# mindspore-lab/minddiffusion

Hardware: AMD Instinct MI355X
Metric: 512x512 txt2img latents/sec (50-step DDIM) (higher is better)
Workload: dtype f16; 1 GPU; SDv2 txt2img 512x512 (64x64 latent), 50-step DDIM, CFG 9.0, batch 1 per GPU (BASELINE.json configs[1]); synthetic seeded weights + synthetic text conditioning; global_batch=1, parallelism=batch-shard x1, hip_graph=True, rccl_world_size=1, broadcast_bytes=0, ddim_steps=50, unet_batch_per_gpu=2, sampler=ddim, cfg_dup_prefix=False

## Files before the change

include/mdx.h:

```cpp
#ifndef MDX_H_
#define MDX_H_

#include <stddef.h>
#include <stdint.h>

#ifdef __cplusplus
extern "C" {
#endif

#define MDX_OK 0
#define MDX_E_INVALID (-1)
#define MDX_E_WORKSPACE (-2)
#define MDX_E_HIP (-3)

typedef void* mdx_stream_t;

int mdx_version(void);
const char* mdx_last_error(void);
int mdx_set_option(const char* name, int value);
int mdx_get_option(const char* name, int* value);

int mdx_nchw_to_nhwc_f16(const float* x, void* y, int B, int C, int H, int W, int Cpad, mdx_stream_t s);
int mdx_nhwc_to_nchw_f32(const void* x, float* y, int B, int C, int H, int W, int Cstride, mdx_stream_t s);

// ... 101 lines not shown

int mdx_groupnorm_from_splitk_f16(const mdx_gemm_desc* prod, const float* gamma, const float* beta, void* y, int groups,
                                  float eps, int silu, mdx_stream_t s);
int mdx_groupnorm_from_splitk_ok(const mdx_gemm_desc* prod, int groups);

int mdx_attention_f16(const void* q, long q_bs, int q_ld, const void* k, long k_bs, int k_ld, const void* vt,
                      long vt_bs, int vt_ld, void* o, long o_bs, int o_ld, int B, int heads, int D, int Nq, int Nk,
                      float scale, mdx_stream_t s);

size_t mdx_attention_ws_bytes(int B, int heads, int D, int Nq, int Nk);
int mdx_attention_splitkv_f16(const void* q, long q_bs, int q_ld, const void* k, long k_bs, int k_ld, const void* vt,
                              long vt_bs, int vt_ld, void* o, long o_bs, int o_ld, int B, int heads, int D, int Nq, int Nk,
                              float scale, int kv_splits, void* ws, size_t ws_bytes, mdx_stream_t s);

typedef struct mdx_st_tail_desc {
    const void* attn_out;
    const void* tok;
    const void* x_in;
    void* out;
    const void* ctx_k;
    const void* ctx_vt;
    const void* wstream;
    const float* vec;
    float* colstats_out;
    void* debug_out;
    int debug_stage;
    int B, tokens;
    int C, heads, dim_head;
    int ctx_len, ctx_cap;
    float scale;
    float ln_eps;
    int tile_rows;
    int warm;
} mdx_st_tail_desc;
#define MDX_ST_DEBUG_COUNT_BARRIERS 100
int mdx_st_tail_sched_barriers(int C, int tile_rows);
int mdx_st_head_sched_barriers(int C, int tile_rows);
int mdx_st_tail_f16(const mdx_st_tail_desc* d, mdx_stream_t s);
int mdx_st_tail_supported(int C, int heads, int dim_head, int tokens_per_sample, int tile_rows);
size_t mdx_st_tail_stream_bytes(int C);

typedef struct mdx_st_head_desc {
    const void* x;
    const float* colstats;
    int nrb;
    const void* wstream;
    const float* vec;
    void* tok;
    void* qk;
    void* vt;
    int vt_ld;
    void* debug_out;
    int debug_stage;
    int B, tokens, C;
    float gn_eps, ln_eps;
    int tile_rows;
    int warm;
} mdx_st_head_desc;
int mdx_st_head_f16(const mdx_st_head_desc* d, mdx_stream_t s);
int mdx_st_head_supported(int C, int tokens_per_sample, int tile_rows);
size_t mdx_st_head_stream_bytes(int C);

int mdx_timestep_embedding_f32(const float* t, float* out, int M, int dim, float max_period, mdx_stream_t s);

int mdx_dense_small_f32(const float* x, int x_ld, const void* w, const float* b, float* out, int out_ld, int M,
                        int N, int K, int act_in, int act_out, mdx_stream_t s);
// ... 143 lines not shown
```

minddiffusion_amd/_lib.py:

```python
import ctypes
import os

_HERE = os.path.dirname(os.path.abspath(__file__))
LIB_PATH = os.environ.get("MDX_LIBRARY") or os.path.join(_HERE, "libmdx.so")

c_void_p = ctypes.c_void_p
c_int = ctypes.c_int
c_uint = ctypes.c_uint
c_long = ctypes.c_long
c_float = ctypes.c_float
c_size_t = ctypes.c_size_t


class MdxError(RuntimeError):
    pass


class GemmDesc(ctypes.Structure):
    _fields_ = [
        ("a", c_void_p), ("a2", c_void_p), ("c1", c_int), ("c2", c_int),
        ("w", c_void_p), ("bias", c_void_p), ("rowbias", c_void_p), ("rowbias_ld", c_int),
        ("residual", c_void_p), ("residual_ld", c_int),
        ("out", c_void_p), ("out_ld", c_int),
        ("B", c_int), ("H", c_int), ("W", c_int), ("N", c_int),
        ("ksize", c_int), ("stride", c_int), ("upsample", c_int),
        ("epilogue", c_int), ("out_mode", c_int), ("splitk", c_int),
        ("workspace", c_void_p), ("workspace_bytes", c_size_t),
        ("out_bs", c_long),
        ("out2", c_void_p), ("out2_ld", c_int), ("n_split", c_int), ("asym_pad", c_int),
        ("stats_out", c_void_p), ("ln_stats", c_void_p), ("ln_s", c_void_p), ("ln_nt", c_int), ("ln_eps", c_float),
        ("colstats_out", c_void_p), ("colstats_cap", c_int), ("defer_reduce", c_int),
        ("tile_m", c_int), ("tile_n", c_int),
        ("gn_colstats", c_void_p), ("gn_gamma", c_void_p), ("gn_beta", c_void_p), ("gn_nrb", c_int), ("gn_silu", c_int),
        ("gn_eps", c_float),
        ("skip_a", c_void_p), ("skip_a2", c_void_p), ("skip_c1", c_int), ("skip_c2", c_int), ("skip_w", c_void_p),
        ("w_frag", c_int), ("stages", c_int), ("w_sub", c_void_p),
        ("xattn_k", c_void_p), ("xattn_vt", c_void_p), ("xattn_len", c_int), ("xattn_cap", c_int), ("xattn_scale", c_float),
        ("act_slope", c_void_p), ("act_slope_n", c_int),
        ("geglu_unit", c_int),
    ]


class StTailDesc(ctypes.Structure):
    _fields_ = [
        ("attn_out", c_void_p), ("tok", c_void_p), ("x_in", c_void_p), ("out", c_void_p),
        ("ctx_k", c_void_p), ("ctx_vt", c_void_p), ("wstream", c_void_p), ("vec", c_void_p),
        ("colstats_out", c_void_p), ("debug_out", c_void_p), ("debug_stage", c_int),
        ("B", c_int), ("tokens", c_int), ("C", c_int), ("heads", c_int), ("dim_head", c_int),
        ("ctx_len", c_int), ("ctx_cap", c_int), ("scale", c_float), ("ln_eps", c_float), ("tile_rows", c_int), ("warm", c_int),
    ]


class StHeadDesc(ctypes.Structure):
    _fields_ = [
        ("x", c_void_p), ("colstats", c_void_p), ("nrb", c_int), ("wstream", c_void_p), ("vec", c_void_p),
        ("tok", c_void_p), ("qk", c_void_p), ("vt", c_void_p), ("vt_ld", c_int), ("debug_out", c_void_p), ("debug_stage", c_int),
        ("B", c_int), ("tokens", c_int), ("C", c_int), ("gn_eps", c_float), ("ln_eps", c_float), ("tile_rows", c_int),
        ("warm", c_int),
    ]


class LoraMergeDesc(ctypes.Structure):
    _fields_ = [
        ("base", c_void_p), ("A", c_void_p), ("B", c_void_p), ("N", c_int), ("K", c_int), ("R", c_int), ("scale", c_float),
        ("gamma", c_void_p), ("beta", c_void_p), ("bias", c_void_p), ("S", c_void_p), ("cb", c_void_p),
        ("dst", c_void_p), ("layout", c_int), ("ld", c_int), ("dst_n0", c_int), ("dst_N", c_int),
        ("piece_stride", c_int), ("piece_offset", c_int),
    ]


EPI_NONE, EPI_GEGLU, EPI_GELU, EPI_QUICKGELU, EPI_PRELU = 0, 1, 2, 3, 4
OUT_ROWMAJOR, OUT_TRANSPOSED, OUT_D2S2 = 0, 1, 2
LORA_ROWMAJOR, LORA_TILED, LORA_FRAG = 0, 1, 2

SIGNATURES = {
    "mdx_version": (c_int, []),
    "mdx_last_error": (ctypes.c_char_p, []),
    "mdx_set_option": (c_int, [ctypes.c_char_p, c_int]),
    "mdx_get_option": (c_int, [ctypes.c_char_p, ctypes.POINTER(c_int)]),
    "mdx_nchw_to_nhwc_f16": (c_int, [c_void_p, c_void_p, c_int, c_int, c_int, c_int, c_int, c_void_p]),
    "mdx_nhwc_to_nchw_f32": (c_int, [c_void_p, c_void_p, c_int, c_int, c_int, c_int, c_int, c_void_p]),
    "mdx_groupnorm_ws_floats": (c_size_t, [c_int, c_int, c_int, c_int]),
# ... 143 lines not shown
```

minddiffusion_amd/csrc/attention.hip:

```cpp
#include "mdx_common.h"

#include <type_traits>
#include <utility>

namespace {

struct AttnParams {
    const f16* q;
    const f16* k;
    const f16* vt;
    f16* o;
    long q_bs, k_bs, vt_bs, o_bs;
    int q_ld, k_ld, vt_ld, o_ld;
    int B, heads, Nq, Nk;
    float scale_log2;
    unsigned k_bytes, vt_bytes;
    int causal;
    int nsplit, qblocks;
    char* ws_part;
    unsigned* tickets;
    int fast_stage;
};

constexpr int BQ = 128;
// ... 852 lines not shown
template <int D, int OCC>
void launch_attn(const AttnParams& p, dim3 grid, hipStream_t st) {
    constexpr int KS = (D + 15) / 16, DT = (D + 31) / 32;
    constexpr int KCH = (2 * KS <= 8) ? 8 : (2 * KS <= 16 ? 16 : 32);
    constexpr size_t stage = (size_t)BKV * KCH * 16 + (size_t)DT * 32 * 128;
    constexpr size_t ostage = (size_t)4 * 32 * (DT * 32 + 8) * 2 + 16;
    constexpr size_t lds = (2 * stage > ostage ? 2 * stage : ostage);
    static MdxPerDeviceOnce attr_once;
    if (attr_once.first()) {
        (void)hipFuncSetAttribute(reinterpret_cast<const void*>(&attn_kernel<D, OCC>),
                                  hipFuncAttributeMaxDynamicSharedMemorySize, (int)lds);
    }
    hipLaunchKernelGGL((attn_kernel<D, OCC>), grid, dim3(256), lds, st, p);
}

constexpr int ATTN_MAX_SPLITS = ATTN_MAX_SPLITS_K;

int attn_cus() {
    static int cus[64] = {};
    int dv = 0;
    if (hipGetDevice(&dv) != hipSuccess || dv < 0 || dv >= 64) return 256;
    if (!cus[dv]) {
        int n = 0;
        cus[dv] = (hipDeviceGetAttribute(&n, hipDeviceAttributeMultiprocessorCount, dv) == hipSuccess && n > 0) ? n : 256;
    }
    return cus[dv];
}

int attn_blocks_per_cu(int D) { return D <= 64 ? (mdx_opt(MDX_OPT_ATTN_OCC3) ? 3 : 2) : (D <= 80 ? 2 : 1); }

int attn_auto_splits(int B, int heads, int D, int Nq, int Nk) {
    const int mode = mdx_opt(MDX_OPT_ATTN_KV_SPLIT);
    const int ntiles = (Nk + BKV - 1) / BKV;
    int cap = mode >= 2 ? ntiles / 2 : ntiles / 24;
    if (cap > ATTN_MAX_SPLITS) cap = ATTN_MAX_SPLITS;
    if (mode == 0 || cap < 2) return 1;
    if (mode >= 2) return mode < cap ? mode : cap;
    const long items = (long)((Nq + BQ - 1) / BQ) * heads * B;
    const long slots = (long)attn_cus() * attn_blocks_per_cu(D);
    long s = slots / items;
    if (s > cap) s = cap;
    return s < 2 ? 1 : (int)s;
}

constexpr long ATTN_TICKET_ITEMS = 16384;
constexpr size_t ATTN_TICKET_BYTES = (size_t)ATTN_TICKET_ITEMS * 4;
size_t attn_part_bytes(int D) { return (size_t)BQ * D * 2 + (size_t)BQ * 8; }

}

static int attention_impl(const void* q, long q_bs, int q_ld, const void* k, long k_bs, int k_ld, const void* vt,
                          long vt_bs, int vt_ld, void* o, long o_bs, int o_ld, int B, int heads, int D, int Nq, int Nk,
                          float scale, int causal, int kv_splits, void* ws, size_t ws_bytes, mdx_stream_t s) {
    MDX_REQUIRE(q && k && vt && o, "mdx_attention_f16: null pointer");
    MDX_REQUIRE(D == 40 || D == 64 || D == 80 || D == 160, "mdx_attention_f16: head dim %d not supported (40/64/80/160)", D);
    MDX_REQUIRE(B > 0 && heads > 0 && Nq > 0 && Nk > 0, "mdx_attention_f16: bad extents");
    MDX_REQUIRE(q_ld % 8 == 0 && k_ld % 8 == 0 && vt_ld % 8 == 0 && o_ld % 8 == 0, "mdx_attention_f16: strides must be multiples of 8");
    MDX_REQUIRE(vt_ld >= Nk, "mdx_attention_f16: vt_ld < Nk");
    AttnParams p{};
    p.q = (const f16*)q;
    p.k = (const f16*)k;
    p.vt = (const f16*)vt;
    p.o = (f16*)o;
    p.q_bs = q_bs; p.k_bs = k_bs; p.vt_bs = vt_bs; p.o_bs = o_bs;
    p.q_ld = q_ld; p.k_ld = k_ld; p.vt_ld = vt_ld; p.o_ld = o_ld;
    p.B = B; p.heads = heads; p.Nq = Nq; p.Nk = Nk;
    p.scale_log2 = scale * 1.4426950408889634f;
    p.causal = causal;
    const size_t kbytes = ((size_t)(Nk - 1) * k_ld + D) * 2;
    const size_t vbytes = ((size_t)(D - 1) * vt_ld + vt_ld) * 2;
    MDX_REQUIRE(kbytes <= 0x80000000ull && vbytes <= 0x80000000ull, "mdx_attention_f16: K/V extent too large");
// ... 97 lines not shown
```

minddiffusion_amd/csrc/stchain.hip:

```cpp
#include "mdx_common.h"

namespace {

typedef unsigned u32x4 __attribute__((ext_vector_type(4)));

struct StTailParams {
    const f16* attn_o;
    const f16* tok;
    const f16* x_in;
    f16* out;
    const f16* kc;
    const f16* vtc;
    const char* wstream;
    const float* vec;
    float* colstats_out;
    f16* dbg;
    int M, HW, TC, ctx_len, heads, nshare, lead;
    float scale_log2, eps;
    int stop_after;
    unsigned wstream_bytes, kc_bytes, vtc_bytes;
};

constexpr int PF = 10;

__device__ __forceinline__ void lds_barrier() {
    asm volatile("s_waitcnt lgkmcnt(0)\n\ts_barrier" ::: "memory");
}

#define LDS_BARRIER() do { lds_barrier(); ++nbar; } while (0)
constexpr int ST_COUNT_BARRIERS = 100;

__device__ __forceinline__ u32x4 wload(const __amdgpu_buffer_rsrc_t rs, unsigned voff, unsigned piece) {
    return __builtin_amdgcn_raw_buffer_load_b128(rs, voff, piece * 1024u, 0);
}

template <int C, int TM, int T>
__device__ __forceinline__ void unit(f32x16 (&acc)[T][TM], const char* abuf_lane, u32x4 (&ring)[PF],
                                     const __amdgpu_buffer_rsrc_t rs, const unsigned voff, unsigned& piece) {
    constexpr int KS = C / 16;
    constexpr int LDB = (C + 8) * 2;
    static_assert((KS * T) % PF == 0, "ring position must be 0 at every unit boundary");
    constexpr int AD = 2;
    f16x8 af[AD + 1][TM];
    f32x16 odd;
#pragma unroll
    for (int r = 0; r < 16; ++r) odd[r] = 0.f;
#pragma unroll
    for (int s = 0; s < AD; ++s)
#pragma unroll
        for (int i = 0; i < TM; ++i) af[s][i] = *reinterpret_cast<const f16x8*>(abuf_lane + i * 32 * LDB + s * 32);
    __builtin_amdgcn_sched_barrier(0);
#pragma unroll
    for (int s = 0; s < KS; ++s) {
// ... 194 lines not shown
                if (dd < D)
                    *reinterpret_cast<f16x4*>(Ab + (rt * 32 + l31) * LDB + (h * D + dd) * 2) =
                        f16x4{(f16)(acc_o[j][4 * g] * inv), (f16)(acc_o[j][4 * g + 1] * inv), (f16)(acc_o[j][4 * g + 2] * inv),
                              (f16)(acc_o[j][4 * g + 3] * inv)};
            }
    }
}

template <int C, int TM, int D, bool LONG>
__global__ __launch_bounds__((C / 32 + 1) * 64) void st_tail_kernel(const StTailParams p) {
    mdx_kernarg_touch<sizeof(StTailParams)>();
    constexpr int NW = C / 32;
    constexpr int NT = NW * 64;
    constexpr int BM = 32 * TM;
    constexpr int LDW = C + 8;
    constexpr int LDB = LDW * 2;
    constexpr int BUF = BM * LDB;
    constexpr int CPR = C / 8;
    constexpr int NH = (TM == 1) ? 2 : 1;
    using V = VecOff<C>;
    extern __shared__ __attribute__((aligned(16))) char smem[];
    char* Xb = smem;
    char* Ab = smem + BUF;
    char* Hb = smem + 2 * BUF;
    float* vec = reinterpret_cast<float*>(smem + (2 + NH) * BUF);
    float2* part = reinterpret_cast<float2*>(vec + V::total);

    int nbar = 0;
    const int tid = threadIdx.x;
    const int lane = tid & 63;
    const int wave = __builtin_amdgcn_readfirstlane(tid >> 6);
    const int hi = lane >> 5, l31 = lane & 31;
    const int m0 = blockIdx.x * BM;
    const int n0 = wave * 32;

    const __amdgpu_buffer_rsrc_t rs_w = make_rsrc(p.wstream, p.wstream_bytes);
    constexpr unsigned PIECES = 3 * (C / 16) + 4 * 3 * (C / 16) + (C / 16);
    if (wave == NW) {
        if (p.nshare <= 0) return;
        constexpr BarSched S = make_sched<C / 16, NH>();
        warmer_wave<NW, PIECES>(p.wstream, S, p.nshare, (unsigned)p.lead, lane);
        return;
    }
    unsigned piece = (unsigned)wave * PIECES;
    const unsigned voff = (unsigned)lane * 16u;
    u32x4 ring[PF];
#pragma unroll
    for (int j = 0; j < PF; ++j) ring[j] = wload(rs_w, voff, piece + j);

    {
        const f16* ga = p.attn_o + (size_t)m0 * C;
        const f16* gx = p.tok + (size_t)m0 * C;
        for (int idx = tid; idx < BM * CPR; idx += NT) {
            const int row = idx / CPR, ch = idx - row * CPR;
            const f16x8 va = *reinterpret_cast<const f16x8*>(ga + (size_t)row * C + ch * 8);
            const f16x8 vx = *reinterpret_cast<const f16x8*>(gx + (size_t)row * C + ch * 8);
            *reinterpret_cast<f16x8*>(Ab + row * LDB + ch * 16) = va;
            *reinterpret_cast<f16x8*>(Xb + row * LDB + ch * 16) = vx;
        }
        for (int idx = tid; idx < V::total / 4; idx += NT)
            reinterpret_cast<float4*>(vec)[idx] = reinterpret_cast<const float4*>(p.vec)[idx];
    }
    LDS_BARRIER();

    const int lane_row_off = l31 * LDB + hi * 16;
    const int epi_off = l31 * LDB + (n0 + 4 * hi) * 2;

    auto dump = [&](const char* buf) {
        LDS_BARRIER();
        for (int idx = tid; idx < BM * CPR; idx += NT) {
            const int row = idx / CPR, ch = idx - row * CPR;
            *reinterpret_cast<f16x8*>(p.dbg + (size_t)(m0 + row) * C + ch * 8) =
                *reinterpret_cast<const f16x8*>(buf + row * LDB + ch * 16);
        }
    };

    auto residual_ln = [&](f32x16 (&acc)[1][TM], const float* bias, const float* gamma, const float* beta) {
        f16x4 th[TM][4];
#pragma unroll
        for (int i = 0; i < TM; ++i) {
            float su = 0.f, sq = 0.f;
#pragma unroll
            for (int g = 0; g < 4; ++g) {
                const float4 bb = *reinterpret_cast<const float4*>(bias + n0 + 8 * g + 4 * hi);
                const f16x4 xr = *reinterpret_cast<const f16x4*>(Xb + epi_off + i * 32 * LDB + g * 16);
// ... 156 lines not shown
    zero_acc(acc1);
    unit<C, TM, 1>(acc1, Ab + lane_row_off, ring, rs_w, voff, piece);
    residual_ln(acc1, vec + V::bo2, vec + V::g3, vec + V::be3);
    if (p.stop_after == 5) { dump(Xb); return; }
    if (p.stop_after == 6) { dump(Ab); return; }

    f32x16 acc2[1][TM];
    zero_acc(acc2);
#pragma unroll 1
    for (int c = 0; c < 4; ++c) {
        f32x16 accg[2][TM];
        zero_acc(accg);
        unit<C, TM, 2>(accg, Ab + lane_row_off, ring, rs_w, voff, piece);
        const float* ba = vec + V::b1 + c * C + n0 + 4 * hi;
        const float* bg = ba + 4 * C;
#pragma unroll
        for (int i = 0; i < TM; ++i)
#pragma unroll
            for (int g = 0; g < 4; ++g) {
                const float4 a4 = *reinterpret_cast<const float4*>(ba + 8 * g);
                const float4 g4 = *reinterpret_cast<const float4*>(bg + 8 * g);
                const float aa[4] = {a4.x, a4.y, a4.z, a4.w}, gg[4] = {g4.x, g4.y, g4.z, g4.w};
                f16x4 hv;
#pragma unroll
                for (int e = 0; e < 4; ++e) hv[e] = (f16)((accg[0][i][4 * g + e] + aa[e]) * gelu_tanh_f(accg[1][i][4 * g + e] + gg[e]));
                *reinterpret_cast<f16x4*>(Hb + (c % NH) * BUF + epi_off + i * 32 * LDB + g * 16) = hv;
            }
        LDS_BARRIER();
        unit<C, TM, 1>(acc2, Hb + (c % NH) * BUF + lane_row_off, ring, rs_w, voff, piece);
        if (NH == 1) LDS_BARRIER();
    }
    {
        f16x8 xin[(BM * CPR + NT - 1) / NT];
        const f16* gx = p.x_in + (size_t)m0 * C;
#pragma unroll
        for (int k = 0; k < (BM * CPR + NT - 1) / NT; ++k) {
            const int idx = tid + k * NT;
            if (idx < BM * CPR) {
                const int row = idx / CPR, ch = idx - row * CPR;
                xin[k] = *reinterpret_cast<const f16x8*>(gx + (size_t)row * C + ch * 8);
            }
        }
#pragma unroll
        for (int i = 0; i < TM; ++i)
#pragma unroll
            for (int g = 0; g < 4; ++g) {
                const float4 bb = *reinterpret_cast<const float4*>(vec + V::b2 + n0 + 8 * g + 4 * hi);
                const f16x4 xr = *reinterpret_cast<const f16x4*>(Xb + epi_off + i * 32 * LDB + g * 16);
                const float b4[4] = {bb.x, bb.y, bb.z, bb.w};
                f16x4 tv;
#pragma unroll
                for (int e = 0; e < 4; ++e) tv[e] = (f16)(acc2[0][i][4 * g + e] + b4[e] + (float)xr[e]);
                *reinterpret_cast<f16x4*>(Ab + epi_off + i * 32 * LDB + g * 16) = tv;
            }
        LDS_BARRIER();
#pragma unroll
        for (int k = 0; k < (BM * CPR + NT - 1) / NT; ++k) {
            const int idx = tid + k * NT;
            if (idx < BM * CPR) {
                const int row = idx / CPR, ch = idx - row * CPR;
                *reinterpret_cast<f16x8*>(Xb + row * LDB + ch * 16) = xin[k];
            }
        }
    }
    if (p.stop_after == 7) { dump(Ab); return; }

    zero_acc(acc1);
// ... 304 lines not shown
    }
    if (p.stop_after == ST_COUNT_BARRIERS && blockIdx.x == 0 && tid == 0) *reinterpret_cast<int*>(p.dbg) = nbar;
}

template <int C, int TM>
void launch_head(const StHeadParams& p, hipStream_t st) {
    constexpr int NW = C / 32, BM = 32 * TM;
    constexpr size_t lds = (size_t)3 * BM * (C + 8) * 2 + (size_t)5 * C * 4 + (size_t)C * 8 + (size_t)NW * BM * 8;
    static_assert(lds <= 160 * 1024, "LDS budget");
    static MdxPerDeviceOnce attr_once;
    if (attr_once.first()) {
        (void)hipFuncSetAttribute(reinterpret_cast<const void*>(&st_head_kernel<C, TM>),
                                  hipFuncAttributeMaxDynamicSharedMemorySize, (int)lds);
    }
    hipLaunchKernelGGL((st_head_kernel<C, TM>), dim3(p.M / BM), dim3((NW + 1) * 64), lds, st, p);
}
}

extern "C" size_t mdx_st_tail_stream_bytes(int C) { return (size_t)(C / 32) * (16 * (C / 16)) * 1024; }

extern "C" int mdx_st_tail_supported(int C, int heads, int dim_head, int tokens_per_sample, int tile_rows) {
    return C == 320 && heads * dim_head == C && (dim_head == 64 || dim_head == 40) && (tile_rows == 32 || tile_rows == 64) &&
           tokens_per_sample > 0 && tokens_per_sample % tile_rows == 0;
}

extern "C" int mdx_st_tail_f16(const mdx_st_tail_desc* d, mdx_stream_t s) {
    MDX_REQUIRE(d && d->attn_out && d->tok && d->x_in && d->out && d->ctx_k && d->ctx_vt && d->wstream && d->vec,
                "mdx_st_tail_f16: null pointer");
    MDX_REQUIRE(mdx_st_tail_supported(d->C, d->heads, d->dim_head, d->tokens, d->tile_rows),
                "mdx_st_tail_f16: unsupported shape C=%d heads=%d d=%d tokens=%d tile_rows=%d", d->C, d->heads, d->dim_head,
                d->tokens, d->tile_rows);
    MDX_REQUIRE(d->B > 0 && d->ctx_len > 0 && d->ctx_len <= d->ctx_cap && d->ctx_cap % 8 == 0 && d->ctx_cap <= 1024,
                "mdx_st_tail_f16: context length %d / capacity %d (capacity: multiple of 8, <= 1024)", d->ctx_len, d->ctx_cap);
    MDX_REQUIRE(d->out != d->attn_out && d->out != d->tok && d->out != d->x_in, "mdx_st_tail_f16: out must not alias an input");
    StTailParams p{};
    p.attn_o = (const f16*)d->attn_out;
    p.tok = (const f16*)d->tok;
    p.x_in = (const f16*)d->x_in;
    p.out = (f16*)d->out;
    p.kc = (const f16*)d->ctx_k;
    p.vtc = (const f16*)d->ctx_vt;
    p.wstream = (const char*)d->wstream;
    p.vec = d->vec;
    p.colstats_out = d->colstats_out;
    p.dbg = (f16*)d->debug_out;
    p.M = d->B * d->tokens;
    p.HW = d->tokens;
    p.TC = d->ctx_cap;
    p.ctx_len = d->ctx_len;
    p.heads = d->heads;
    {
        const int per_xcd = (p.M / d->tile_rows) / 8;
        p.nshare = (d->debug_out || d->warm == 0 || per_xcd < 4) ? 0 : (per_xcd > 32 ? 32 : per_xcd);
        p.lead = 80;
        if (d->warm > 1) {
            p.lead = d->warm / 100;
            if (p.nshare > 0 && d->warm % 100 > 0 && d->warm % 100 < p.nshare) p.nshare = d->warm % 100;
        }
    }
    p.scale_log2 = d->scale * 1.4426950408889634f;
    p.eps = d->ln_eps;
    p.stop_after = d->debug_out ? d->debug_stage : 0;
    p.wstream_bytes = (unsigned)mdx_st_tail_stream_bytes(d->C);
    p.kc_bytes = (unsigned)((size_t)d->ctx_cap * d->C * 2);
    p.vtc_bytes = (unsigned)((size_t)d->C * d->ctx_cap * 2);
    hipStream_t st = (hipStream_t)s;
    const bool lng = d->ctx_len > 96;
    if (d->dim_head == 64) {
        if (d->tile_rows == 64) { if (lng) launch_tail<320, 2, 64, true>(p, st); else launch_tail<320, 2, 64, false>(p, st); }
        else { if (lng) launch_tail<320, 1, 64, true>(p, st); else launch_tail<320, 1, 64, false>(p, st); }
    } else {
        if (d->tile_rows == 64) { if (lng) launch_tail<320, 2, 40, true>(p, st); else launch_tail<320, 2, 40, false>(p, st); }
        else { if (lng) launch_tail<320, 1, 40, true>(p, st); else launch_tail<320, 1, 40, false>(p, st); }
    }
    MDX_LAUNCH_CHECK("mdx_st_tail_f16");
    return MDX_OK;
}

extern "C" int mdx_st_tail_sched_barriers(int C, int tile_rows) {
// ... 48 lines not shown
```

minddiffusion_amd/ldm/modules/diffusionmodules/openaimodel.py:

```python
import ctypes
import math
import os
import re
import weakref

import torch

from .... import ops
from ...._lib import MdxError
from ....planner import PlanBuilder, round_up, capture_or_eager
from ....loader import WeightLoader, named_layers

f16, f32 = torch.float16, torch.float32

LORA_PREFIXES = ("tk_delta_", "mindpet_delta_")
_LORA_KEY = re.compile(r"^(.*)\.(" + "|".join(LORA_PREFIXES) + r")lora_([ab])$")
_LORA_TARGETS = ("to_q", "to_k", "to_v", "to_out.0")


def is_lora_key(name):
    return _LORA_KEY.match(name) is not None


class UNetModel:
# ... 491 lines not shown
        B, C, H, W = x.shape
        if C != self.in_channels:
            raise MdxError(f"UNetModel: expected {self.in_channels} input channels, got {C}")
        if context is None:
            if getattr(self, "_selfctx_bad", None) is None:
                self._selfctx_bad = sorted({l[2] * l[3] for _, l in named_layers(self)
                                            if l[0] == "st" and l[2] * l[3] != self.context_dim})
            bad = self._selfctx_bad
            if bad:
                raise MdxError(f"UNetModel: context=None makes attn2 attend to its own input (attention.py:133), which needs "
                               f"context_dim == transformer width; context_dim={self.context_dim}, widths {bad}")
            P = self._plan(B, H, W, _selfctx=True)
        else:
            P = self._plan(B, H, W)
            self._ensure_context(P, context)
        P.x_static.copy_(x)
        if temb is not None:
            if temb.shape[-1] != self._emb_total or temb.dtype != f32:
                raise MdxError(f"UNetModel: temb must be fp32 [.., {self._emb_total}] rows of time_embedding_table()")
            P.emb_all.copy_(temb)
        else:
            P.t_static.copy_(timesteps.to(device=self.device, dtype=f32) if isinstance(timesteps, torch.Tensor)
                             else torch.as_tensor(timesteps, dtype=f32, device=self.device))
            if y is not None:
                yy = torch.as_tensor(y).to(device=self.device, dtype=torch.long).reshape(-1)
                if yy.shape[0] != B:
                    raise MdxError(f"UNetModel: y has {yy.shape[0]} labels for a batch of {B}")
                if int(yy.min()) < 0 or int(yy.max()) >= self.num_classes:
                    raise MdxError(f"UNetModel: class label outside [0, {self.num_classes})")
                P.y_static.copy_(yy)
            for op in P.main[:P.temb_ops]:
                op()
        dup = self._dup_body(P) if (cfg_dup and context is not None and y is None) else None
        if dup is not None and ops.get_option("unet_cfg_dup_check"):
            hb = B // 2
            same = torch.equal(P.x_static[:hb], P.x_static[hb:]) and torch.equal(P.emb_all[:hb], P.emb_all[hb:])
            if not same:
                raise MdxError("UNetModel: cfg_dup=True, but the two halves of the batch do not carry the same x / timesteps")
        if self.use_graph and not P.graph_failed:
            if dup is not None:
                if P.dup_graph is None:
                    self._capture(P, dup)
                if P.dup_graph is not None:
                    P.dup_graph.replay()
                    return P.eps_nhwc
            if P.graph is None:
                self._capture(P)
            if P.graph is not None:
                P.graph.replay()
                return P.eps_nhwc
        body = dup if dup is not None else P.main[P.temb_ops:]
        for op in body:
            op()
        self.last_launch_count = P.temb_ops + len(body)
        return P.eps_nhwc

    def _dup_body(self, P):
        mn = ops.get_option("unet_cfg_dup")
        if not mn or P.B < mn or P.B % 2 or P.ck is None:
            return None
        if hasattr(P, "dup_body"):
            return P.dup_body
        P.dup_body = None
        h = P.B // 2
        PA = self._plan(h, P.H, P.W)
        if PA.ck is None:
            return None
        late = "op2" in P.ck and "op2" in PA.ck and len(P.ck["live2"]) == len(PA.ck["live2"])
        ko, kl = ("op2", "live2") if late else ("op", "live")
        ib, ic = P.main.index(P.ck[ko]), P.main.index(P.ck["conv_in"])
        ja, jc = PA.main.index(PA.ck[ko]), PA.main.index(PA.ck["conv_in"])
        xin_a, xin_b = PA.ck["xin"], P.ck["xin"]
        copies = [lambda: xin_a.copy_(xin_b[:h]), lambda: PA.emb_all.copy_(P.emb_all[:h])]
        spread = []
        for src, dst in zip(PA.ck[kl], P.ck[kl]):
            if not (dst.shape[0] == 2 * src.shape[0] and dst.shape[1:] == src.shape[1:] and dst.dtype == src.dtype):
                raise MdxError(f"UNetModel: guidance-duplicate prefix: live tensors of the two plans do not pair up "
                               f"({tuple(src.shape)} vs {tuple(dst.shape)})")
            spread.append(lambda src=src, dst=dst, k=src.shape[0]: (dst[:k].copy_(src), dst[k:].copy_(src)))
        P.dup_half = PA
        P.dup_body = P.main[P.temb_ops:ic + 1] + copies + PA.main[jc:ja + 1] + spread + P.main[ib + 1:]
        small = {"kind": "small", "flops": 0, "launches": 1, "info": "guidance-duplicate prefix: copy"}
        P.dup_meta = (P.meta[P.temb_ops:ic + 1] + [dict(small) for _ in copies] + PA.meta[jc:ja + 1]
                      + [dict(small, launches=2) for _ in spread] + P.meta[ib + 1:])
        return P.dup_body

    def _capture(self, P, dup=None):
        body = dup if dup is not None else P.main[P.temb_ops:]
        graphs = capture_or_eager([body])
        if graphs is None:
            P.graph, P.graph_failed = None, True
        elif dup is not None:
            P.dup_graph = graphs[0]
        else:
            P.graph = graphs[0]
        if graphs is not None:
            P.graph_ctx_len = P.ctx_len

    def construct(self, x, timesteps=None, context=None, y=None):
        eps = self.forward_nhwc(x, timesteps, context, y=y)
        B, _, H, W = x.shape
        return ops.nhwc_to_nchw(eps, self.final_channels, H, W)

    __call__ = construct
    forward = construct


class _HeadNotWired(Exception):
    """A fused SpatialTransformer head / GroupNorm-in-conv launch did not get its column statistics (UNetModel._plan)."""


class _UNetPlanner(PlanBuilder):

    def __init__(self, net, B, H, W, fuse_head, selfctx):
        super().__init__(net.device, B, track_producers=True)
        self.net, self.w, self.H, self.W = net, net.w, H, W
        self.fuse_head, self.selfctx = fuse_head, selfctx
        self.TC = net.max_context_len
# ... 244 lines not shown
        forced = ops.get_option("unet_st_tail")
        cands = [forced] if forced in (32, 64) else ([] if forced == 0 else [64, 32])
        for r in cands:
            if not ops.st_tail_supported(heads * dh, heads, dh, n, r):
                continue
            blocks = self.B * n // r
            if forced in (32, 64) or (r == 64 and blocks >= 512) or (r == 32 and blocks >= 192):
                return r
        return 0

    def head_rows(self, t, x, n, heads, dh):
        if not self.fuse_head or (t + "head.stream") not in self.w or ops.get_option("unet_st_head") == 0:
            return 0
        r = self.tail_rows(t, n, heads, dh)
        if not r or not ops.st_head_supported(heads * dh, n, r) or self.producer.get(x.data_ptr()) is None:
            return 0
        return r

    def context_kv(self, t, inner):
        kc = torch.zeros((self.B, self.TC, inner), dtype=f16, device=self.dev)
        vtc = torch.zeros((self.B, inner, self.TC), dtype=f16, device=self.dev)
        self.ctx_kv[t] = (kc, vtc)
        return kc, vtc

    def fused_tail(self, t, rows_t, o, tok, x, ch, inner, heads, dh, n):
        w, B, P, TC = self.w, self.B, self.P, self.TC
        kc, vtc = self.context_kv(t, inner)
        out = self.get((B, n, ch))
        td = ops.make_st_tail_desc(o, tok, x, out, kc, vtc, w[t + "tail.stream"], w[t + "tail.vec"], B, n, ch, heads,
                                   dh, 1, TC, tile_rows=rows_t)
        self.tails.append(td)
        td._bufs = (o, tok, x, out, kc, vtc)
        self.producer[out.data_ptr()] = td

        def run_tail(td=td):
            td.ctx_len = P.ctx_len
            ops.st_tail_run(td)
        self.emit(run_tail, "gemm", 2 * B * n * 16 * inner * inner + 4 * B * heads * n * self.ctx_flops * dh, 1,
                  f"st_tail M={B * n} C={inner} rows={rows_t} (to_out1..proj_out fused)")
        return out

    def stats_buf(self, rows, width):
        if (rows, width) not in self.ln_stats:
            self.ln_stats[(rows, width)] = torch.zeros((rows, width // 64, 2), dtype=f32, device=self.dev)
        return self.ln_stats[(rows, width)]

    def vt_buffer(self, n, inner):
        if n % 8 == 0:
            return self.get((self.B, inner, n))
        t_ = torch.zeros((self.B, inner, round_up(n, 8)), dtype=f16, device=self.dev)
        self.ragged_vt.append(t_)
        return t_

    def vt_release(self, t_):
        if not any(t_ is r for r in self.ragged_vt):
            self.release(t_)

    def first_self_attention(self):
        return "op" not in self.ck and "conv_in" in self.ck and len(self.hs) == 1

    def fused_transformer(self, t0, rows_h, x, ch, heads, dh, n):
        w, B = self.w, self.B
        inner = heads * dh
        tok = self.get((B, n, inner))
        qk = self.get((B, n, 2 * inner))
        vt = self.get((B, inner, n))
        hd = ops.make_st_head_desc(x, x, 1, w[t0 + "head.stream"], w[t0 + "head.vec"], tok, qk, vt, n, B, n, ch,
                                   tile_rows=rows_h)
        hd.colstats = 0
        self.heads_fused.append(hd)
        hd._bufs = (x, tok, qk, vt)
        self.gn_calls.append(dict(x1=x, x2=None, head=hd, meta=len(self.meta), film=False,
                                  prod=(self.producer.get(x.data_ptr()), None)))
        self.emit(lambda hd=hd: ops.st_head_run(hd), "gemm", 2 * B * n * 4 * inner * inner, 1,
                  f"st_head M={B * n} C={inner} rows={rows_h} (GroupNorm..q|k|v fused)")
        o = self.get((B, n, inner))
        self.attention(qk, vt, o, heads, dh, f"self B={B} h={heads} N={n} d={dh}", split_kv=True)
        if self.first_self_attention():
            self.ck.update(op=self.main[-1], live=(x, tok, o))
        out = self.fused_tail(t0, self.tail_rows(t0, n, heads, dh), o, tok, x, ch, inner, heads, dh, n)
        self.release(qk, vt, tok, o)
        return out

    def transformer(self, pre, x, ch, heads, dh, h, wd):
        net, w, B, P, TC = self.net, self.w, self.B, self.P, self.TC
        dense, emit, selfctx = self.dense, self.emit, self.selfctx
        n = h * wd
        inner = heads * dh
        scale = dh ** -0.5
        t0 = pre + "transformer_blocks.0."
        rows_h = self.head_rows(t0, x, n, heads, dh)
        if rows_h:
            return self.fused_transformer(t0, rows_h, x, ch, heads, dh, n)
        a = self.get((B, n, ch))
        self.gn(x, None, w[pre + "norm.g"], w[pre + "norm.b"], 1e-6, False, a)
        st = self.stats_buf(B * n, inner) if (t0 + "attn2.q.s") in w else None
        fold1 = st is not None and (t0 + "attn1.qkv.s") in w

        def consumer(name):
            return dict(bias=w[name + ".cb"], ln_stats=st, ln_s=w[name + ".s"], ln_eps=1e-5)

        def layernorm(src, t, norm, ln):
            emit(lambda: ops.layernorm(src, w[t + norm + ".g"], w[t + norm + ".b"], 1e-5, out=ln), "layernorm")
        tok = dense(a, B, n, ch, inner, w[pre + "proj_in.w"], bias=w[pre + "proj_in.b"], stats_out=st if fold1 else None)
        pf = ops.get_option("unet_gn_proj_fuse")
        if (self.fuse_head and pf and n >= pf and n % 64 == 0 and ch % 64 == 0 and ch <= 2560
                and self.producer.get(x.data_ptr()) is not None):
            self.gn_calls[-1]["proj"] = dict(desc=self.descs[-1], meta=len(self.meta) - 1)
        self.release(a)
        for k in range(net.transformer_depth):
            t = pre + f"transformer_blocks.{k}."
            last = k == net.transformer_depth - 1
            ln = self.get((B, n, inner))
            if not fold1:
                layernorm(tok, t, "norm1", ln)
            vt = self.vt_buffer(n, inner)
            nv = vt.shape[2]
            if (t + "attn1.qkv.w") in w:
                qk = self.get((B, n, 2 * inner))
                self.gemm(a=tok if fold1 else ln, w=w[t + "attn1.qkv.w"], N=3 * inner, B=B, H=n, W=1, c1=inner, out=qk,
                          out_ld=2 * inner, out2=vt, out2_ld=nv, n_split=2 * inner,
                          **(consumer(t + "attn1.qkv") if fold1 else {}))
            else:
                qk = dense(ln, B, n, inner, 2 * inner, w[t + "attn1.qk.w"])
                dense(ln, B, n, inner, inner, w[t + "attn1.v.w"], out=vt, out_ld=nv, out_mode=ops.OUT_TRANSPOSED)
            o = ln
            self.attention(qk, vt, o, heads, dh, f"self B={B} h={heads} N={n} d={dh}", split_kv=True)
            first = self.first_self_attention()
            rows_t = self.tail_rows(t, n, heads, dh)
            if first:
                self.ck.update(op=self.main[-1], live=(x, tok, o))
            if rows_t:
                out = self.fused_tail(t, rows_t, o, tok, x, ch, inner, heads, dh, n)
                self.release(qk); self.vt_release(vt); self.release(tok, ln)
                return out
            tok2 = dense(o, B, n, inner, inner, w[t + "attn1.o.w"], bias=w[t + "attn1.o.b"], residual=tok, stats_out=st)
            if first:
                self.ck.update(op2=self.main[-1], live2=(x, tok2) + (() if st is None else (st,)))
            self.release(qk); self.vt_release(vt); self.release(tok)
            xfuse = (ops.get_option("unet_xattn_fuse") and not selfctx and dh == 64 and TC <= 1024 and TC % 8 == 0
                     and n % 64 == 0)
            xkw = {}
            if xfuse:
                kc, vtc = self.context_kv(t, inner)
                xkw = dict(tile_n=64, splitk=1, tile_m=0 if n % 128 == 0 else 64, xattn_k=kc, xattn_vt=vtc, xattn_len=TC,
                           xattn_cap=TC, xattn_scale=scale, out=o, out_ld=inner)
            if st is None:
                layernorm(tok2, t, "norm2", ln)
                q2 = dense(ln, B, n, inner, inner, w[t + "attn2.q.w"], **xkw)
            else:
                q2 = dense(tok2, B, n, inner, inner, w[t + "attn2.q.w"], **consumer(t + "attn2.q"), **xkw)
                if selfctx:
                    layernorm(tok2, t, "norm2", ln)
            if xfuse:
                self.xattn_descs.append(self.descs[-1])
                self.meta[-1]["flops"] += 4 * B * heads * n * self.ctx_flops * dh
                self.meta[-1]["info"] += f" +cross-attention h={heads} d={dh}"
                q2 = None
            if selfctx:
                k2 = dense(ln, B, n, inner, inner, w[t + "attn2.k.w"])
                v2t = self.vt_buffer(n, inner)
                nv2 = v2t.shape[2]
                dense(ln, B, n, inner, inner, w[t + "attn2.v.w"], out=v2t, out_ld=nv2, out_mode=ops.OUT_TRANSPOSED)
                self.attn_ws_need = max(self.attn_ws_need, ops.attention_ws_bytes(B, heads, dh, n, n))
                emit(lambda q2=q2, k2=k2, v2t=v2t, o=o, nv2=nv2: ops.attention(
                    q2.data_ptr(), k2.data_ptr(), v2t.data_ptr(), o.data_ptr(), B, heads, dh, n, n, scale,
# ... 98 lines not shown
```

minddiffusion_amd/ops.py:

```python
import ctypes
import math
import os

import numpy as np
import torch

from . import _lib
from ._lib import GemmDesc, EPI_NONE, EPI_GEGLU, EPI_GELU, EPI_QUICKGELU, OUT_ROWMAJOR, OUT_TRANSPOSED
from ._lib import EPI_PRELU, OUT_D2S2

f16 = torch.float16
f32 = torch.float32


_OPTIONS = {"unet_st_tail": int(os.environ.get("MDX_UNET_ST_TAIL", "-1")),
            "unet_st_head": int(os.environ.get("MDX_UNET_ST_HEAD", "-1")),
            "unet_conv_stream": int(os.environ.get("MDX_UNET_CONV_STREAM", "128")),
            "gn_colstats_fold": int(os.environ.get("MDX_GN_COLSTATS_FOLD", "0")),
            "unet_gn_splitk_fuse": int(os.environ.get("MDX_UNET_GN_SPLITK_FUSE", "256")),
            "unet_conv_stream_w4": int(os.environ.get("MDX_UNET_CONV_STREAM_W4", "0")),
            "unet_skip_fuse": int(os.environ.get("MDX_UNET_SKIP_FUSE", "1")),
            "unet_gn_conv_fuse": int(os.environ.get("MDX_UNET_GN_CONV_FUSE", "0")),
            "unet_tune_first_use": int(os.environ.get("MDX_UNET_TUNE_FIRST_USE", "0")),
            "unet_subpixel_upsample": int(os.environ.get("MDX_UNET_SUBPIXEL_UPSAMPLE", "1")),
            "unet_gn_proj_fuse": int(os.environ.get("MDX_UNET_GN_PROJ_FUSE", "0")),
            "unet_xattn_fuse": int(os.environ.get("MDX_UNET_XATTN_FUSE", "1")),
            "unet_cfg_dup": int(os.environ.get("MDX_UNET_CFG_DUP", "4")),
            "unet_cfg_dup_check": int(os.environ.get("MDX_UNET_CFG_DUP_CHECK", "0")),
            "unet_ff_proj_fuse": int(os.environ.get("MDX_UNET_FF_PROJ_FUSE", "640")),
            "glide_qkv_merge": int(os.environ.get("MDX_GLIDE_QKV_MERGE", "1")),
            "glide_gn_qkv_fuse": int(os.environ.get("MDX_GLIDE_GN_QKV_FUSE", "0"))}


def set_option(name, value):
    if name in _OPTIONS:
        _OPTIONS[name] = int(value)
        return
    _lib.check(_lib.load().mdx_set_option(name.encode(), int(value)), "mdx_set_option")


def get_option(name):
    if name in _OPTIONS:
        return _OPTIONS[name]
    out = ctypes.c_int(0)
    _lib.check(_lib.load().mdx_get_option(name.encode(), ctypes.byref(out)), "mdx_get_option")
    return int(out.value)


def capture_graph(ops_list):
    import gc
    g = torch.cuda.CUDAGraph()
    gc.collect()
    was_enabled = gc.isenabled()
    gc.disable()
    try:
        with torch.cuda.graph(g):
            for op in ops_list:
                op()
    finally:
        if was_enabled:
# ... 967 lines not shown
def pack_frag_weight(w2d):
    N, K = w2d.shape
    assert N % 32 == 0 and K % 16 == 0
    t = w2d.to(f16).reshape(N // 32, 32, K // 16, 2, 8).permute(0, 2, 3, 1, 4)
    return t.reshape(N // 32, K // 16, 512).contiguous()


def pack_st_tail(wo1, wq2, wo2, w1, w2, wpo, bo1, g2, be2, bo2, g3, be3, b1, b2, bpo):
    C = wo1.shape[0]
    NW, KS = C // 32, C // 16
    f = pack_frag_weight
    fo1, fq2, fo2, fpo = f(wo1), f(wq2), f(wo2), f(wpo)
    f1 = f(w1)
    f2 = f(w2)
    parts = [fo1, fq2, fo2]
    for c in range(4):
        a = f1[c * NW:(c + 1) * NW]
        g = f1[4 * C // 32 + c * NW:4 * C // 32 + (c + 1) * NW]
        parts.append(torch.stack([a, g], 2).reshape(NW, 2 * KS, 512))
        parts.append(f2[:, c * KS:(c + 1) * KS])
    parts.append(fpo)
    stream = torch.cat(parts, 1).contiguous()
    assert stream.shape == (NW, 16 * KS, 512)
    vec = torch.cat([v.to(f32).reshape(-1) for v in (bo1, g2, be2, bo2, g3, be3, b1, b2, bpo)]).contiguous()
    assert vec.numel() == 16 * C
    return stream, vec


def st_tail_supported(C, heads, dim_head, tokens, tile_rows):
    return bool(_lib.load().mdx_st_tail_supported(int(C), int(heads), int(dim_head), int(tokens), int(tile_rows)))


def make_st_tail_desc(attn_out, tok, x_in, out, ctx_k, ctx_vt, stream, vec, B, tokens, C, heads, dim_head, ctx_len, ctx_cap,
                      tile_rows=64, ln_eps=1e-5, colstats_out=None, debug_out=None, debug_stage=0):
    d = _lib.StTailDesc()
    d.attn_out, d.tok, d.x_in, d.out = attn_out.data_ptr(), tok.data_ptr(), x_in.data_ptr(), out.data_ptr()
    d.ctx_k, d.ctx_vt, d.wstream, d.vec = ctx_k.data_ptr(), ctx_vt.data_ptr(), stream.data_ptr(), vec.data_ptr()
    d.colstats_out = 0 if colstats_out is None else colstats_out.data_ptr()
    d.debug_out = 0 if debug_out is None else debug_out.data_ptr()
    d.debug_stage = int(debug_stage)
    d.B, d.tokens, d.C, d.heads, d.dim_head = int(B), int(tokens), int(C), int(heads), int(dim_head)
    d.ctx_len, d.ctx_cap = int(ctx_len), int(ctx_cap)
    d.scale, d.ln_eps, d.tile_rows = float(dim_head) ** -0.5, float(ln_eps), int(tile_rows)
    d.warm = int(os.environ.get("MDX_ST_TAIL_WARM", "1"))
    return d


def st_tail_run(desc):
    _lib.check(_lib.load().mdx_st_tail_f16(ctypes.byref(desc), _stream()), "mdx_st_tail_f16")


def pack_st_head(wpi, wq, wk, wv, gn_g, gn_b, bpi, g1, be1):
    f = pack_frag_weight
    stream = torch.cat([f(wpi), f(wq), f(wk), f(wv)], 1).contiguous()
    vec = torch.cat([t.to(f32).reshape(-1) for t in (gn_g, gn_b, bpi, g1, be1)]).contiguous()
    return stream, vec


def st_head_supported(C, tokens, tile_rows):
    return bool(_lib.load().mdx_st_head_supported(int(C), int(tokens), int(tile_rows)))


def make_st_head_desc(x, colstats, nrb, stream, vec, tok, qk, vt, vt_ld, B, tokens, C, tile_rows=32, gn_eps=1e-6, ln_eps=1e-5,
                      debug_out=None, debug_stage=0):
    d = _lib.StHeadDesc()
    d.x, d.colstats, d.nrb = x.data_ptr(), colstats.data_ptr(), int(nrb)
    d.wstream, d.vec = stream.data_ptr(), vec.data_ptr()
    d.tok, d.qk, d.vt, d.vt_ld = tok.data_ptr(), qk.data_ptr(), vt.data_ptr(), int(vt_ld)
    d.debug_out = 0 if debug_out is None else debug_out.data_ptr()
    d.debug_stage = int(debug_stage)
    d.B, d.tokens, d.C = int(B), int(tokens), int(C)
    d.gn_eps, d.ln_eps, d.tile_rows = float(gn_eps), float(ln_eps), int(tile_rows)
    d.warm = int(os.environ.get("MDX_ST_TAIL_WARM", "1"))
    return d


def st_head_run(desc):
# ... 44 lines not shown
```

Baseline: 5.258 latents/s.

## Let fused ST tail read half-batch sources directly, dropping CFG-dup spread copies

Adds a src_rows field to the fused spatial-transformer tail so rows beyond src_rows wrap modulo, letting the tail read the half-batch prefix outputs directly instead of first copying them into both halves of the full batch. The guidance-duplicate path points the tail at the half-plan buffers and drops the spread copy ops, with an option to keep the old spread behaviour. Separately, attention KV-split selection uses a lower tile threshold when there are fewer work items than CUs, giving more splits for small grids. The pointer switching between dup and non-dup paths adds state that must be kept consistent with captured graphs.

```diff
diff --git a/include/mdx.h b/include/mdx.h
--- a/include/mdx.h
+++ b/include/mdx.h
@@ -157,6 +157,7 @@
     float ln_eps;
     int tile_rows;
     int warm;
+    int src_rows;
 } mdx_st_tail_desc;
 #define MDX_ST_DEBUG_COUNT_BARRIERS 100
 int mdx_st_tail_sched_barriers(int C, int tile_rows);
diff --git a/minddiffusion_amd/_lib.py b/minddiffusion_amd/_lib.py
--- a/minddiffusion_amd/_lib.py
+++ b/minddiffusion_amd/_lib.py
@@ -48,6 +48,7 @@
         ("colstats_out", c_void_p), ("debug_out", c_void_p), ("debug_stage", c_int),
         ("B", c_int), ("tokens", c_int), ("C", c_int), ("heads", c_int), ("dim_head", c_int),
         ("ctx_len", c_int), ("ctx_cap", c_int), ("scale", c_float), ("ln_eps", c_float), ("tile_rows", c_int), ("warm", c_int),
+        ("src_rows", c_int),
     ]
 
 
diff --git a/minddiffusion_amd/csrc/attention.hip b/minddiffusion_amd/csrc/attention.hip
--- a/minddiffusion_amd/csrc/attention.hip
+++ b/minddiffusion_amd/csrc/attention.hip
@@ -908,11 +908,15 @@
 int attn_auto_splits(int B, int heads, int D, int Nq, int Nk) {
     const int mode = mdx_opt(MDX_OPT_ATTN_KV_SPLIT);
     const int ntiles = (Nk + BKV - 1) / BKV;
-    int cap = mode >= 2 ? ntiles / 2 : ntiles / 24;
+#ifndef MDX_ATTN_LONE_MIN_TILES
+#define MDX_ATTN_LONE_MIN_TILES 20
+#endif
+    const long items = (long)((Nq + BQ - 1) / BQ) * heads * B;
+    const int min_tiles = (mode == 1 && items < attn_cus()) ? MDX_ATTN_LONE_MIN_TILES : 24;
+    int cap = mode >= 2 ? ntiles / 2 : ntiles / min_tiles;
     if (cap > ATTN_MAX_SPLITS) cap = ATTN_MAX_SPLITS;
     if (mode == 0 || cap < 2) return 1;
     if (mode >= 2) return mode < cap ? mode : cap;
-    const long items = (long)((Nq + BQ - 1) / BQ) * heads * B;
     const long slots = (long)attn_cus() * attn_blocks_per_cu(D);
     long s = slots / items;
     if (s > cap) s = cap;
diff --git a/minddiffusion_amd/csrc/stchain.hip b/minddiffusion_amd/csrc/stchain.hip
--- a/minddiffusion_amd/csrc/stchain.hip
+++ b/minddiffusion_amd/csrc/stchain.hip
@@ -19,6 +19,7 @@
     float scale_log2, eps;
     int stop_after;
     unsigned wstream_bytes, kc_bytes, vtc_bytes;
+    int src_rows;
 };
 
 constexpr int PF = 10;
@@ -279,6 +280,7 @@
     const int wave = __builtin_amdgcn_readfirstlane(tid >> 6);
     const int hi = lane >> 5, l31 = lane & 31;
     const int m0 = blockIdx.x * BM;
+    const int ms = m0 < p.src_rows ? m0 : (int)((unsigned)m0 % (unsigned)p.src_rows);
     const int n0 = wave * 32;
 
     const __amdgpu_buffer_rsrc_t rs_w = make_rsrc(p.wstream, p.wstream_bytes);
@@ -296,8 +298,8 @@
     for (int j = 0; j < PF; ++j) ring[j] = wload(rs_w, voff, piece + j);
 
     {
-        const f16* ga = p.attn_o + (size_t)m0 * C;
-        const f16* gx = p.tok + (size_t)m0 * C;
+        const f16* ga = p.attn_o + (size_t)ms * C;
+        const f16* gx = p.tok + (size_t)ms * C;
         for (int idx = tid; idx < BM * CPR; idx += NT) {
             const int row = idx / CPR, ch = idx - row * CPR;
             const f16x8 va = *reinterpret_cast<const f16x8*>(ga + (size_t)row * C + ch * 8);
@@ -520,7 +522,7 @@
     }
     {
         f16x8 xin[(BM * CPR + NT - 1) / NT];
-        const f16* gx = p.x_in + (size_t)m0 * C;
+        const f16* gx = p.x_in + (size_t)ms * C;
 #pragma unroll
         for (int k = 0; k < (BM * CPR + NT - 1) / NT; ++k) {
             const int idx = tid + k * NT;
@@ -891,7 +893,18 @@
                 d->tokens, d->tile_rows);
     MDX_REQUIRE(d->B > 0 && d->ctx_len > 0 && d->ctx_len <= d->ctx_cap && d->ctx_cap % 8 == 0 && d->ctx_cap <= 1024,
                 "mdx_st_tail_f16: context length %d / capacity %d (capacity: multiple of 8, <= 1024)", d->ctx_len, d->ctx_cap);
-    MDX_REQUIRE(d->out != d->attn_out && d->out != d->tok && d->out != d->x_in, "mdx_st_tail_f16: out must not alias an input");
+    const int M = d->B * d->tokens;
+    MDX_REQUIRE(d->src_rows >= 0 && d->src_rows <= M && d->src_rows % d->tile_rows == 0 && (d->src_rows == 0 || M % d->src_rows == 0),
+                "mdx_st_tail_f16: src_rows=%d must be 0 or a multiple of tile_rows=%d that divides M=%d", d->src_rows, d->tile_rows, M);
+    const int src_rows = d->src_rows ? d->src_rows : M;
+    {
+        const char* o0 = (const char*)d->out;
+        const char* o1 = o0 + (size_t)M * d->C * 2;
+        const size_t in_bytes = (size_t)src_rows * d->C * 2;
+        const char* ins[3] = {(const char*)d->attn_out, (const char*)d->tok, (const char*)d->x_in};
+        for (const char* i0 : ins)
+            MDX_REQUIRE(i0 + in_bytes <= o0 || o1 <= i0, "mdx_st_tail_f16: out must not alias an input");
+    }
     StTailParams p{};
     p.attn_o = (const f16*)d->attn_out;
     p.tok = (const f16*)d->tok;
@@ -903,7 +916,8 @@
     p.vec = d->vec;
     p.colstats_out = d->colstats_out;
     p.dbg = (f16*)d->debug_out;
-    p.M = d->B * d->tokens;
+    p.M = M;
+    p.src_rows = src_rows;
     p.HW = d->tokens;
     p.TC = d->ctx_cap;
     p.ctx_len = d->ctx_len;
diff --git a/minddiffusion_amd/ldm/modules/diffusionmodules/openaimodel.py b/minddiffusion_amd/ldm/modules/diffusionmodules/openaimodel.py
--- a/minddiffusion_amd/ldm/modules/diffusionmodules/openaimodel.py
+++ b/minddiffusion_amd/ldm/modules/diffusionmodules/openaimodel.py
@@ -547,6 +547,7 @@
             for op in P.main[:P.temb_ops]:
                 op()
         dup = self._dup_body(P) if (cfg_dup and context is not None and y is None) else None
+        self._point_dup_tail(P, dup is not None)
         if dup is not None and ops.get_option("unet_cfg_dup_check"):
             hb = B // 2
             same = torch.equal(P.x_static[:hb], P.x_static[hb:]) and torch.equal(P.emb_all[:hb], P.emb_all[hb:])
@@ -574,9 +575,12 @@
         mn = ops.get_option("unet_cfg_dup")
         if not mn or P.B < mn or P.B % 2 or P.ck is None:
             return None
-        if hasattr(P, "dup_body"):
+        keep = ops.get_option("unet_cfg_dup_spread")
+        if hasattr(P, "dup_body") and P.dup_keep_spread == keep:
+            self._point_dup_tail(P, P.dup_body is not None)
             return P.dup_body
-        P.dup_body = None
+        self._point_dup_tail(P, False)
+        P.dup_body, P.dup_graph, P.dup_tail, P.dup_keep_spread = None, None, None, keep
         h = P.B // 2
         PA = self._plan(h, P.H, P.W)
         if PA.ck is None:
@@ -593,12 +597,25 @@
                 raise MdxError(f"UNetModel: guidance-duplicate prefix: live tensors of the two plans do not pair up "
                                f"({tuple(src.shape)} vs {tuple(dst.shape)})")
             spread.append(lambda src=src, dst=dst, k=src.shape[0]: (dst[:k].copy_(src), dst[k:].copy_(src)))
+        tail = P.ck.get("tail")
+        if not late and not keep and tail is not None and ib + 1 < len(P.main) and P.main[ib + 1] is tail[0]:
+            xa, toka, oa = PA.ck[kl]
+            P.dup_tail = tail[1]
+            P.dup_src = (oa.data_ptr(), toka.data_ptr(), xa.data_ptr(), xa.shape[0] * xa.shape[1])
+            spread = []
+            self._point_dup_tail(P, True)
         P.dup_half = PA
         P.dup_body = P.main[P.temb_ops:ic + 1] + copies + PA.main[jc:ja + 1] + spread + P.main[ib + 1:]
         small = {"kind": "small", "flops": 0, "launches": 1, "info": "guidance-duplicate prefix: copy"}
         P.dup_meta = (P.meta[P.temb_ops:ic + 1] + [dict(small) for _ in copies] + PA.meta[jc:ja + 1]
                       + [dict(small, launches=2) for _ in spread] + P.meta[ib + 1:])
         return P.dup_body
+
+    @staticmethod
+    def _point_dup_tail(P, dup):
+        td = getattr(P, "dup_tail", None)
+        if td is not None:
+            td._src = P.dup_src if dup else td._own
 
     def _capture(self, P, dup=None):
         body = dup if dup is not None else P.main[P.temb_ops:]
@@ -909,9 +926,11 @@
         self.tails.append(td)
         td._bufs = (o, tok, x, out, kc, vtc)
         self.producer[out.data_ptr()] = td
+        td._own = td._src = (o.data_ptr(), tok.data_ptr(), x.data_ptr(), 0)
 
         def run_tail(td=td):
             td.ctx_len = P.ctx_len
+            td.attn_out, td.tok, td.x_in, td.src_rows = td._src
             ops.st_tail_run(td)
         self.emit(run_tail, "gemm", 2 * B * n * 16 * inner * inner + 4 * B * heads * n * self.ctx_flops * dh, 1,
                   f"st_tail M={B * n} C={inner} rows={rows_t} (to_out1..proj_out fused)")
@@ -953,9 +972,12 @@
                   f"st_head M={B * n} C={inner} rows={rows_h} (GroupNorm..q|k|v fused)")
         o = self.get((B, n, inner))
         self.attention(qk, vt, o, heads, dh, f"self B={B} h={heads} N={n} d={dh}", split_kv=True)
-        if self.first_self_attention():
+        first = self.first_self_attention()
+        if first:
             self.ck.update(op=self.main[-1], live=(x, tok, o))
         out = self.fused_tail(t0, self.tail_rows(t0, n, heads, dh), o, tok, x, ch, inner, heads, dh, n)
+        if first:
+            self.ck["tail"] = (self.main[-1], self.tails[-1])
         self.release(qk, vt, tok, o)
         return out
 
@@ -1009,6 +1031,8 @@
                 self.ck.update(op=self.main[-1], live=(x, tok, o))
             if rows_t:
                 out = self.fused_tail(t, rows_t, o, tok, x, ch, inner, heads, dh, n)
+                if first:
+                    self.ck["tail"] = (self.main[-1], self.tails[-1])
                 self.release(qk); self.vt_release(vt); self.release(tok, ln)
                 return out
             tok2 = dense(o, B, n, inner, inner, w[t + "attn1.o.w"], bias=w[t + "attn1.o.b"], residual=tok, stats_out=st)
diff --git a/minddiffusion_amd/ops.py b/minddiffusion_amd/ops.py
--- a/minddiffusion_amd/ops.py
+++ b/minddiffusion_amd/ops.py
@@ -26,6 +26,7 @@
             "unet_gn_proj_fuse": int(os.environ.get("MDX_UNET_GN_PROJ_FUSE", "0")),
             "unet_xattn_fuse": int(os.environ.get("MDX_UNET_XATTN_FUSE", "1")),
             "unet_cfg_dup": int(os.environ.get("MDX_UNET_CFG_DUP", "4")),
+            "unet_cfg_dup_spread": int(os.environ.get("MDX_UNET_CFG_DUP_SPREAD", "0")),
             "unet_cfg_dup_check": int(os.environ.get("MDX_UNET_CFG_DUP_CHECK", "0")),
             "unet_ff_proj_fuse": int(os.environ.get("MDX_UNET_FF_PROJ_FUSE", "640")),
             "glide_qkv_merge": int(os.environ.get("MDX_GLIDE_QKV_MERGE", "1")),
@@ -1059,7 +1060,7 @@
 
 
 def make_st_tail_desc(attn_out, tok, x_in, out, ctx_k, ctx_vt, stream, vec, B, tokens, C, heads, dim_head, ctx_len, ctx_cap,
-                      tile_rows=64, ln_eps=1e-5, colstats_out=None, debug_out=None, debug_stage=0):
+                      tile_rows=64, ln_eps=1e-5, colstats_out=None, debug_out=None, debug_stage=0, src_rows=0):
     d = _lib.StTailDesc()
     d.attn_out, d.tok, d.x_in, d.out = attn_out.data_ptr(), tok.data_ptr(), x_in.data_ptr(), out.data_ptr()
     d.ctx_k, d.ctx_vt, d.wstream, d.vec = ctx_k.data_ptr(), ctx_vt.data_ptr(), stream.data_ptr(), vec.data_ptr()
@@ -1070,6 +1071,7 @@
     d.ctx_len, d.ctx_cap = int(ctx_len), int(ctx_cap)
     d.scale, d.ln_eps, d.tile_rows = float(dim_head) ** -0.5, float(ln_eps), int(tile_rows)
     d.warm = int(os.environ.get("MDX_ST_TAIL_WARM", "1"))
+    d.src_rows = int(src_rows)
     return d
 
 
```

Result: no change. 5.256 latents/s (median of 2 runs) (-0.0%).
